# aai-institute/USFlows

Measured on AMD Instinct MI355X. Metric: log_prob samples/sec (whole node), 32-layer 784-dim flow, batch 65536, higher is better.
Workload: dtype f32 (GEMMs as bf16x3 split on the bf16 MFMA: 24 significant bits, fp32 accumulate); 1 GPU; BASELINE cfg2: USFlow in_dims=[784], 32 additive coupling blocks, ConditionalDenseNN[256, 256]+LeakyReLU(0.01), lu_transform=1, householder=0, affine_conjugation=False, Laplace(0,1) base; log_prob of 65536 rows per GPU (65536 over 1 GPU(s)) resident in HBM; conditioned synthetic parameters (seed 100, alpha 0.1); rows_per_gpu=65536, global_rows=65536, parallelism=dp1 (single GPU: no collective), fused_coupling=True, gemm_mode=bf16x3, merge_affine=auto -> False; probe (accepted, element-wise, L1) []

## Files before the change

### usflows_amd/csrc/usf_coupling_planes.hip

```cpp
#include <stdlib.h>

#include "usf_common.h"

namespace usf {

typedef __bf16 cp_bf16x8 __attribute__((ext_vector_type(8)));
typedef _Float16 cp_f16x8 __attribute__((ext_vector_type(8)));
#define USF_CP_F16_GUARD 65000.0f

template <int NPL> struct CPlanes;
template <> struct CPlanes<3> {
  typedef cp_bf16x8 vec;
  static __device__ __forceinline__ f32x4 mfma(vec a, vec b, f32x4 c) { return __builtin_amdgcn_mfma_f32_16x16x32_bf16(a, b, c, 0, 0, 0); }
  static __device__ __forceinline__ void split(const f32x4 x0, const f32x4 x1, vec (&o)[3]) {
#pragma unroll
    for (int j = 0; j < 8; ++j) {
      const float x = (j < 4) ? x0[j & 3] : x1[j & 3];
      const __bf16 h = (__bf16)x;
      const float r = x - (float)h;
      const __bf16 m = (__bf16)r;
      o[0][j] = h; o[1][j] = m; o[2][j] = (__bf16)(r - (float)m);
    }
  }
  static __device__ __forceinline__ void split1(const float x, const int j, vec (&o)[3]) {
    const __bf16 h = (__bf16)x;
    const float r = x - (float)h;
    const __bf16 m = (__bf16)r;
    o[0][j] = h; o[1][j] = m; o[2][j] = (__bf16)(r - (float)m);
  }
  static __device__ __forceinline__ void mm(f32x4& acc, const vec (&w)[3], const vec (&a)[3]) {
    acc = mfma(w[2], a[0], acc); acc = mfma(w[1], a[1], acc); acc = mfma(w[0], a[2], acc);
    acc = mfma(w[1], a[0], acc); acc = mfma(w[0], a[1], acc); acc = mfma(w[0], a[0], acc);
  }
};
template <> struct CPlanes<2> {
  typedef cp_f16x8 vec;
  static __device__ __forceinline__ f32x4 mfma(vec a, vec b, f32x4 c) { return __builtin_amdgcn_mfma_f32_16x16x32_f16(a, b, c, 0, 0, 0); }
  static __device__ __forceinline__ void split(const f32x4 x0, const f32x4 x1, vec (&o)[2]) {
#pragma unroll
    for (int j = 0; j < 8; ++j) {
      const float x = (j < 4) ? x0[j & 3] : x1[j & 3];
      const _Float16 h = (_Float16)x;
      o[0][j] = h; o[1][j] = (_Float16)(x - (float)h);
    }
  }
  static __device__ __forceinline__ void split1(const float x, const int j, vec (&o)[2]) {
    const _Float16 h = (_Float16)x;
    o[0][j] = h; o[1][j] = (_Float16)(x - (float)h);
  }
  static __device__ __forceinline__ void mm(f32x4& acc, const vec (&w)[2], const vec (&a)[2]) {
    acc = mfma(w[1], a[0], acc); acc = mfma(w[0], a[1], acc); acc = mfma(w[0], a[0], acc);
  }
};

struct CplPArgs {
  char* z; int z_nkb, npanels, M;
  int kb_p0, nk_p, kb_t0, nk_t;
  const char* Win; int64_t ld_in, pl_in; const float* b_in;
  const char* Whid[2]; int64_t ld_hid, pl_hid; const float* b_hid[2];
  const char* Wout; int64_t ld_out, pl_out; const float* b_out;
  float sign, slope; int act;
  int32_t* range_flag;
  unsigned long long* dbg;
  char* hout[2]; const char* gate[2];
  const float* ctx; int ctx_stride; const float* w_ctx; const float* b_ctx;
};

#ifdef USF_STAMP
#define CSTAMP(v) unsigned long long v = __builtin_amdgcn_s_memtime(); __builtin_amdgcn_sched_barrier(0)
#else
#define CSTAMP(v)
#endif

template <int NPL, int NH, int MODE = 0, bool CTX = false>
__global__ __launch_bounds__(512, 2) void coupling_planes_kernel(const CplPArgs p) {
  typedef CPlanes<NPL> PT;
  typedef typename PT::vec vec8;
  constexpr int T = 16;
  constexpr int HP = 16 * T;
  constexpr int KS = T / 2;
  constexpr int NT = 512;
  constexpr int SLOTS = NPL * 4 * HP;
  constexpr int NST = SLOTS / NT;
  constexpr int NPP = NST / NPL;
  constexpr int NC = HP / 8;
  constexpr int NPR = (NPL == 3) ? 6 : 3;
#ifndef USF_CP_AHEAD
#define USF_CP_AHEAD 3
#endif
  constexpr int AHEAD = USF_CP_AHEAD;
  __shared__ __attribute__((aligned(16))) float lds[2][SLOTS * 4];

  const int tid = threadIdx.x;
  const int lane = tid & 63;
  const int wave = tid >> 6;
  const int lj = lane & 15, lg = lane >> 4;
  const int panel = blockIdx.x * 8 + wave;
  const int panc = min(panel, p.npanels - 1);
  const bool live = panel < p.npanels;
  const bool live_z = CTX ? (live && 16 * panel + lj < p.M) : live;
  const f32x4 zero4 = {0.f, 0.f, 0.f, 0.f};
  constexpr unsigned CHB = NPL * 1024u;
  const size_t zbase = ((size_t)panc * p.z_nkb) * CHB + (size_t)lane * 16;

  int kdst[NPP];
  unsigned krow[NPP];
#pragma unroll
  for (int i = 0; i < NPP; ++i) {
    const int idx = tid + NT * i;
    const int r = idx >> 2, c = idx & 3;
    kdst[i] = 4 * (c * HP + (r ^ (2 * c)));
    krow[i] = (unsigned)r;
  }
  auto issue_k = [&](const char* W, int64_t ld, int64_t pl, int k0, f32x4 (&st)[NST]) {
#pragma unroll
    for (int q = 0; q < NPL; ++q)
#pragma unroll
      for (int i = 0; i < NPP; ++i)
        st[q * NPP + i] = *reinterpret_cast<const f32x4*>(W + 2 * (q * pl + (int64_t)krow[i] * ld + k0 + 8 * ((tid + NT * i) & 3)));
  };
  auto store_k = [&](int buf, const f32x4 (&st)[NST]) {
#pragma unroll
    for (int q = 0; q < NPL; ++q)
#pragma unroll
      for (int i = 0; i < NPP; ++i) *reinterpret_cast<f32x4*>(&lds[buf][q * 16 * HP + kdst[i]]) = st[q * NPP + i];
  };
  auto n_rc = [&](int i, int& r, int& c) { const int idx = tid + NT * i; r = idx / NC; c = idx % NC; };
  auto issue_n = [&](const char* W, int64_t ld, int64_t pl, int n0, f32x4 (&st)[NST]) {
#pragma unroll
    for (int q = 0; q < NPL; ++q)
#pragma unroll
      for (int i = 0; i < NPP; ++i) {
        int r, c; n_rc(i, r, c);
        st[q * NPP + i] = *reinterpret_cast<const f32x4*>(W + 2 * (q * pl + (int64_t)(n0 + r) * ld + 8 * c));
      }
  };
  auto store_n = [&](int buf, const f32x4 (&st)[NST]) {
#pragma unroll
    for (int q = 0; q < NPL; ++q)
#pragma unroll
      for (int i = 0; i < NPP; ++i) {
        int r, c; n_rc(i, r, c);
        *reinterpret_cast<f32x4*>(&lds[buf][4 * ((q * NC + c) * 32 + (r ^ (2 * (c & 7))))]) = st[q * NPP + i];
      }
  };

  f32x4 X1[T], X2[T];
#pragma unroll
  for (int t = 0; t < T; ++t) X1[t] = *reinterpret_cast<const f32x4*>(p.b_in + t * 16 + 4 * lg);
  if (CTX) {
// ... 221 lines not shown
#endif
  if (NPL == 2 && p.range_flag && bad && live && (16 * panel + lj) < p.M) atomicOr(p.range_flag, 1);
#undef CP_PIN_SLAB
}



#ifdef USF_STAMP
unsigned long long* g_cdbg = nullptr;
#endif

int coupling_planes_ctx(const usf_coupling_planes_desc* d, const float* ctx, int64_t ctx_stride, const float* w_ctx,
                        const float* b_ctx, hipStream_t stream) {
  if (!d) { set_error("usf_coupling_planes: null descriptor"); return -1; }
  if (ctx) {
    if (d->act == USF_ACT_GATE) { set_error("usf_coupling_planes_ctx: USF_ACT_GATE takes no context (the context enters no data gradient)"); return -2; }
    if (ctx_stride != 0 && ctx_stride != 1) { set_error("usf_coupling_planes_ctx: ctx_stride must be 0 or 1 (got %lld)", (long long)ctx_stride); return -2; }
    if (!w_ctx || !b_ctx || !aligned16(w_ctx) || !aligned16(b_ctx)) {
      set_error("usf_coupling_planes_ctx: w_ctx / b_ctx must be [256] fp32 vectors, 16-byte aligned");
      return -2;
    }
  }
  if (d->M < 0 || d->M > 0x7fffffff || d->z_nkb <= 0 || d->n_hidden < 1 || d->n_hidden > 3 || d->nk_p <= 0 || d->nk_t <= 0 ||
      d->kb_p0 < 0 || d->kb_t0 < 0 || d->kb_p0 + d->nk_p > d->z_nkb || d->kb_t0 + d->nk_t > d->z_nkb) {
    set_error("usf_coupling_planes: bad sizes / block ranges");
    return -2;
  }
  if (d->M == 0) return 0;
  if (d->format != USF_PLANES_BF16X3 && d->format != USF_PLANES_F16X2) { set_error("usf_coupling_planes: unknown format %d", d->format); return -2; }
  if (!d->z || !d->W_in || !d->W_out || !d->b_in || !d->b_out) { set_error("usf_coupling_planes: null pointer"); return -1; }
  for (int i = 0; i + 1 < d->n_hidden; ++i)
    if (!d->W_hid[i] || !d->b_hid[i]) { set_error("usf_coupling_planes: hidden layer %d missing", i); return -1; }
  if (d->hidden_padded != 256) { set_error("usf_coupling_planes: weights must be padded to a hidden width of 256 (got %d)", d->hidden_padded); return -2; }
  if (d->ldw_in < 32 * d->nk_p || (d->n_hidden > 1 && d->ldw_hid < 256) || d->ldw_out < 256 || (d->ldw_in & 7) || (d->ldw_hid & 7) ||
      (d->ldw_out & 7) || !aligned16(d->z) || !aligned16(d->W_in) || !aligned16(d->W_out) || !aligned16(d->b_in) || !aligned16(d->b_out)) {
    set_error("usf_coupling_planes: weight-image contract violated (ldw_in >= 32 nk_p, ldw_hid / ldw_out >= 256, multiples of 8, 16-byte aligned)");
    return -2;
  }
  const int64_t npl = d->format == USF_PLANES_F16X2 ? 2 : 3;
  const int64_t npanels = (d->M + 15) / 16;
  if (2 * npl * d->w_in_plane >= (1LL << 40)) { set_error("usf_coupling_planes: operand too large"); return -3; }
  CplPArgs a;
  a.z = reinterpret_cast<char*>(d->z); a.z_nkb = (int)d->z_nkb; a.npanels = (int)npanels; a.M = (int)d->M;
  a.kb_p0 = (int)d->kb_p0; a.nk_p = (int)d->nk_p; a.kb_t0 = (int)d->kb_t0; a.nk_t = (int)d->nk_t;
  a.Win = reinterpret_cast<const char*>(d->W_in); a.ld_in = d->ldw_in; a.pl_in = d->w_in_plane; a.b_in = d->b_in;
  for (int i = 0; i < 2; ++i) {
    const bool used = i + 1 < d->n_hidden;
    a.Whid[i] = reinterpret_cast<const char*>(used ? d->W_hid[i] : d->W_in);
    a.b_hid[i] = used ? d->b_hid[i] : d->b_in;
  }
  a.ld_hid = d->ldw_hid; a.pl_hid = d->w_hid_plane;
  a.Wout = reinterpret_cast<const char*>(d->W_out); a.ld_out = d->ldw_out; a.pl_out = d->w_out_plane; a.b_out = d->b_out;
  a.sign = d->sign; a.slope = d->slope; a.act = d->act; a.range_flag = d->range_flag;
  a.ctx = ctx; a.ctx_stride = (int)ctx_stride; a.w_ctx = w_ctx; a.b_ctx = b_ctx;
  a.dbg = nullptr;
#ifdef USF_STAMP
  a.dbg = g_cdbg;
#endif
  const dim3 grid((unsigned)((npanels + 7) / 8));
  const bool want_h = d->hidden_out[0] != nullptr || d->hidden_out[1] != nullptr;
  const bool gated = d->act == USF_ACT_GATE;
  if (d->act != USF_ACT_NONE && d->act != USF_ACT_LEAKY_RELU && !gated) { set_error("usf_coupling_planes: bad act %d", d->act); return -2; }
  for (int i = 0; i < 2; ++i) { a.hout[i] = nullptr; a.gate[i] = nullptr; }
  if (want_h || gated) {
    if (npl != 3 || d->n_hidden > 2) { set_error("usf_coupling_planes: hidden_out / USF_ACT_GATE need the bf16x3 format and n_hidden <= 2"); return -2; }
    if (gated && !want_h) { set_error("usf_coupling_planes: USF_ACT_GATE needs hidden_out (the gradients at the hidden pre-activations)"); return -2; }
    for (int i = 0; i < d->n_hidden; ++i) {
      if (!d->hidden_out[i] || !aligned16(d->hidden_out[i]) || (gated && (!d->gate[i] || !aligned16(d->gate[i])))) {
        set_error("usf_coupling_planes: hidden_out[l] (and gate[l] with USF_ACT_GATE) must be set for every hidden layer, 16-byte aligned");
        return -2;
      }
      a.hout[i] = reinterpret_cast<char*>(d->hidden_out[i]);
      a.gate[i] = reinterpret_cast<const char*>(gated ? d->gate[i] : nullptr);
    }
    const dim3 block(512);
#define USF_CPT(NH_, MODE_) hipLaunchKernelGGL((coupling_planes_kernel<3, NH_, MODE_>), grid, block, 0, stream, a)
#define USF_CPTC(NH_) hipLaunchKernelGGL((coupling_planes_kernel<3, NH_, 1, true>), grid, block, 0, stream, a)
    if (gated) { if (d->n_hidden == 1) USF_CPT(1, 2); else USF_CPT(2, 2); }
    else if (ctx) { if (d->n_hidden == 1) USF_CPTC(1); else USF_CPTC(2); }
    else { if (d->n_hidden == 1) USF_CPT(1, 1); else USF_CPT(2, 1); }
#undef USF_CPTC
#undef USF_CPT
    return check_launch("usf_coupling_planes");
  }
  const dim3 block(512);
#define USF_CPL(NPL_, NH_) hipLaunchKernelGGL((coupling_planes_kernel<NPL_, NH_>), grid, block, 0, stream, a)
#define USF_CPLC(NPL_, NH_) hipLaunchKernelGGL((coupling_planes_kernel<NPL_, NH_, 0, true>), grid, block, 0, stream, a)
  if (ctx) {
    if (npl == 2) {
      switch (d->n_hidden) { case 1: USF_CPLC(2, 1); break; case 2: USF_CPLC(2, 2); break; default: USF_CPLC(2, 3); break; }
    } else {
      switch (d->n_hidden) { case 1: USF_CPLC(3, 1); break; case 2: USF_CPLC(3, 2); break; default: USF_CPLC(3, 3); break; }
    }
  } else if (npl == 2) {
    switch (d->n_hidden) { case 1: USF_CPL(2, 1); break; case 2: USF_CPL(2, 2); break; default: USF_CPL(2, 3); break; }
  } else {
    switch (d->n_hidden) { case 1: USF_CPL(3, 1); break; case 2: USF_CPL(3, 2); break; default: USF_CPL(3, 3); break; }
  }
#undef USF_CPLC
#undef USF_CPL
  return check_launch("usf_coupling_planes");
}

int coupling_planes(const usf_coupling_planes_desc* d, hipStream_t stream) { return coupling_planes_ctx(d, nullptr, 0, nullptr, nullptr, stream); }

}
// ... 1 lines not shown
```

### usflows_amd/csrc/usf_planes.hip

```cpp
#include <stdlib.h>

#include "usf_common.h"

namespace usf {

typedef __bf16 bf16x8 __attribute__((ext_vector_type(8)));
typedef _Float16 f16x8 __attribute__((ext_vector_type(8)));
#define USF_F16_GUARD 65000.0f
#define USF_PL_LOAD_A(ptr) (*(ptr))
#define USF_PL_STORE_C(v, ptr) (*(ptr) = (v))

template <int NPL> struct Planes;
template <> struct Planes<3> {
  typedef bf16x8 vec;
  static __device__ __forceinline__ f32x4 mfma(vec a, vec b, f32x4 c) { return __builtin_amdgcn_mfma_f32_16x16x32_bf16(a, b, c, 0, 0, 0); }
  static __device__ __forceinline__ void split(const float (&x)[8], vec (&o)[3]) {
#pragma unroll
    for (int j = 0; j < 8; ++j) {
      const __bf16 h = (__bf16)x[j];
      const float r = x[j] - (float)h;
      const __bf16 m = (__bf16)r;
      const float r2 = r - (float)m;
      o[0][j] = h; o[1][j] = m; o[2][j] = (__bf16)r2;
    }
  }
};
template <> struct Planes<2> {
  typedef f16x8 vec;
  static __device__ __forceinline__ f32x4 mfma(vec a, vec b, f32x4 c) { return __builtin_amdgcn_mfma_f32_16x16x32_f16(a, b, c, 0, 0, 0); }
  static __device__ __forceinline__ void split(const float (&x)[8], vec (&o)[2]) {
#pragma unroll
    for (int j = 0; j < 8; ++j) {
      const _Float16 h = (_Float16)x[j];
      const float r = x[j] - (float)h;
      o[0][j] = h; o[1][j] = (_Float16)r;
    }
  }
};

__host__ __device__ __forceinline__ int plane_feature_of_slot(int s) { return 16 * ((s & 7) >> 2) + 4 * (s >> 3) + (s & 3); }

template <int NPL>
__global__ __launch_bounds__(256) void pack_planes_kernel(const float* __restrict__ src, int64_t ld, int M, int npanels,
                                                          int nkb, const int32_t* __restrict__ idx,
                                                          const float* __restrict__ pre_div,
                                                          const float* __restrict__ pre_sub, char* __restrict__ dst,
                                                          int32_t* __restrict__ range_flag) {
  typedef Planes<NPL> PT;
  const int lane = threadIdx.x & 63;
  const int lj = lane & 15, lg = lane >> 4;
  const int64_t chunk = (int64_t)blockIdx.x * 4 + (threadIdx.x >> 6);
  if (chunk >= (int64_t)npanels * nkb) return;
  const int p = (int)(chunk / nkb), kb = (int)(chunk % nkb);
  const int row = 16 * p + lj;
  float x[8];
#pragma unroll
  for (int u = 0; u < 8; ++u) {
    const int l = 32 * kb + 16 * (u >> 2) + 4 * lg + (u & 3);
    const int c = idx[l];
    float v = 0.f;
    if (c >= 0 && row < M) {
      v = src[(int64_t)row * ld + c];
      if (pre_div) v = v / pre_div[l];
      if (pre_sub) v = v - pre_sub[l];
    }
    x[u] = v;
  }
  if (NPL == 2 && range_flag) {
    bool bad = false;
#pragma unroll
    for (int u = 0; u < 8; ++u) bad = bad || !(fabsf(x[u]) < USF_F16_GUARD);
    if (bad) atomicOr(range_flag, 1);
  }
  typename PT::vec o[NPL];
  PT::split(x, o);
  char* out = dst + (chunk * NPL) * 1024 + lane * 16;
#pragma unroll
  for (int q = 0; q < NPL; ++q) *reinterpret_cast<typename PT::vec*>(out + q * 1024) = o[q];
}

template <int NPL, bool GRAD>
__global__ __launch_bounds__(256) void pack_planes_rows_kernel(const float* __restrict__ src, int64_t ld, int M, int nkb, int src_cols,
                                                               const int32_t* __restrict__ idx, const float* __restrict__ pre_div,
                                                               const float* __restrict__ pre_sub, char* __restrict__ dst,
                                                               int32_t* __restrict__ range_flag, const float* __restrict__ row_weight,
                                                               const float* __restrict__ loc, const float* __restrict__ scale, int grad_base,
                                                               int vec) {
  typedef Planes<NPL> PT;
  extern __shared__ float tile[];
  const int S = src_cols + 1;
  const int L = 32 * nkb;
  int* const t_idx = reinterpret_cast<int*>(tile + 16 * S);
  float* const t_div = tile + 16 * S + L;
  float* const t_sub = t_div + L;
  const int tid = threadIdx.x, lane = tid & 63, wave = tid >> 6;
  const int p = blockIdx.x;
  for (int e = tid; e < L; e += 256) {
    t_idx[e] = idx[e];
    t_div[e] = pre_div ? pre_div[e] : 1.0f;
    t_sub[e] = pre_sub ? pre_sub[e] : 0.0f;
  }
  auto xform = [&](float v, int c, float w) {
    if (!GRAD) return v;
    const float t = v - loc[c];
    const float sg = (float)((t > 0.f) - (t < 0.f));
    const float g = (grad_base == 1 + USF_BASE_LAPLACE) ? -sg / scale[c] : -t / (scale[c] * scale[c]);
    return g * w;
  };
  if (vec) {
    const int c4n = src_cols >> 2;
    for (int e = tid; e < 16 * c4n; e += 256) {
      const int r = e / c4n, c = 4 * (e - r * c4n);
      const int row = 16 * p + r;
      f32x4 v = {0.f, 0.f, 0.f, 0.f};
      float w = 0.f;
      if (row < M) {
        v = *reinterpret_cast<const f32x4*>(src + (int64_t)row * ld + c);
        if (GRAD) w = row_weight[row];
      }
#pragma unroll
      for (int q = 0; q < 4; ++q) tile[r * S + c + q] = (row < M) ? xform(v[q], c + q, w) : 0.f;
    }
    for (int e = tid; e < 16 * (src_cols & 3); e += 256) {
      const int r = e / (src_cols & 3), c = (src_cols & ~3) + e % (src_cols & 3);
      const int row = 16 * p + r;
      tile[r * S + c] = (row < M) ? xform(src[(int64_t)row * ld + c], c, GRAD ? row_weight[row] : 0.f) : 0.f;
    }
  } else {
    for (int e = tid; e < 16 * src_cols; e += 256) {
      const int r = e / src_cols, c = e - r * src_cols;
      const int row = 16 * p + r;
      tile[r * S + c] = (row < M) ? xform(src[(int64_t)row * ld + c], c, GRAD ? row_weight[row] : 0.f) : 0.f;
    }
  }
  __syncthreads();
  const int lj = lane & 15, lg = lane >> 4;
  const bool row_live = 16 * p + lj < M;
  const bool has_div = pre_div != nullptr, has_sub = pre_sub != nullptr;
  bool bad = false;
  for (int kb = wave; kb < nkb; kb += 4) {
    float x[8];
#pragma unroll
    for (int u = 0; u < 8; ++u) {
      const int l = 32 * kb + 16 * (u >> 2) + 4 * lg + (u & 3);
      const int c = t_idx[l];
      float v = 0.f;
      if (c >= 0 && row_live) {
        v = tile[lj * S + c];
        if (has_div) v = v / t_div[l];
        if (has_sub) v = v - t_sub[l];
      }
      x[u] = v;
    }
    if (NPL == 2) {
#pragma unroll
      for (int u = 0; u < 8; ++u) bad = bad || !(fabsf(x[u]) < USF_F16_GUARD);
    }
    typename PT::vec o[NPL];
    PT::split(x, o);
    char* out = dst + ((int64_t)((int64_t)p * nkb + kb) * NPL) * 1024 + lane * 16;
#pragma unroll
    for (int q = 0; q < NPL; ++q) *reinterpret_cast<typename PT::vec*>(out + q * 1024) = o[q];
  }
  if (NPL == 2 && range_flag && bad) atomicOr(range_flag, 1);
}

int pack_planes(const usf_pack_planes_desc* d, hipStream_t stream) {
  if (!d) { set_error("usf_pack_planes_f32: null descriptor"); return -1; }
  if (d->M < 0 || d->nkb <= 0 || d->M > 0x7fffffff || d->nkb > 0x7fffff || d->ld < 1) { set_error("usf_pack_planes_f32: bad sizes"); return -2; }
  if (d->M == 0) return 0;
  if (!d->src || !d->idx || !d->planes) { set_error("usf_pack_planes_f32: null pointer"); return -1; }
  if (!aligned16(d->planes)) { set_error("usf_pack_planes_f32: planes must be 16-byte aligned"); return -2; }
  if (d->format != USF_PLANES_BF16X3 && d->format != USF_PLANES_F16X2) { set_error("usf_pack_planes_f32: unknown format %d", d->format); return -2; }
  const int64_t npanels = (d->M + 15) / 16;
  const int64_t chunks = npanels * d->nkb;
  const int64_t blocks = (chunks + 3) / 4;
  if (blocks > 0x7fffffffLL) { set_error("usf_pack_planes_f32: grid too large"); return -3; }
  if (d->grad_base != 0) {
    if (d->src_cols <= 0 || !d->row_weight || !d->loc || !d->scale || d->format != USF_PLANES_BF16X3 ||
        (d->grad_base != 1 + USF_BASE_LAPLACE && d->grad_base != 1 + USF_BASE_NORMAL)) {
      set_error("usf_pack_planes_f32: grad_base needs src_cols, row_weight, loc, scale, the bf16x3 format and a Laplace / Normal base");
      return -2;
    }
  }
  const int rows_env = (int)tuning("pack_rows", 1);
  const size_t lds = ((size_t)16 * (size_t)(d->src_cols + 1) + (size_t)3 * 32 * (size_t)d->nkb) * sizeof(float);
  if (d->src_cols > 0 && d->src_cols <= d->ld && lds <= 65536 && (rows_env || d->grad_base != 0)) {
    const int vec = (aligned16(d->src) && (d->ld & 3) == 0) ? 1 : 0;
    char* out = reinterpret_cast<char*>(d->planes);
#define USF_PPR(NPL_, GRAD_) hipLaunchKernelGGL((pack_planes_rows_kernel<NPL_, GRAD_>), dim3((unsigned)npanels), dim3(256), lds, stream, d->src, \
                             d->ld, (int)d->M, (int)d->nkb, (int)d->src_cols, d->idx, d->pre_div, d->pre_sub, out, d->range_flag,      \
                             d->row_weight, d->loc, d->scale, (int)d->grad_base, vec)
    if (d->grad_base != 0) USF_PPR(3, true);
    else if (d->format == USF_PLANES_F16X2) USF_PPR(2, false);
    else USF_PPR(3, false);
#undef USF_PPR
    return check_launch("usf_pack_planes_f32");
  }
  if (d->grad_base != 0) { set_error("usf_pack_planes_f32: grad_base needs 16 (src_cols + 1) floats to fit 64 KB of LDS"); return -2; }
  if (d->format == USF_PLANES_F16X2)
    hipLaunchKernelGGL(pack_planes_kernel<2>, dim3((unsigned)blocks), dim3(256), 0, stream, d->src, d->ld, (int)d->M, (int)npanels,
                       (int)d->nkb, d->idx, d->pre_div, d->pre_sub, reinterpret_cast<char*>(d->planes), d->range_flag);
  else
    hipLaunchKernelGGL(pack_planes_kernel<3>, dim3((unsigned)blocks), dim3(256), 0, stream, d->src, d->ld, (int)d->M, (int)npanels,
                       (int)d->nkb, d->idx, d->pre_div, d->pre_sub, reinterpret_cast<char*>(d->planes), d->range_flag);
  return check_launch("usf_pack_planes_f32");
}

struct PlArgs {
  const char* A; const char* Wp; const float* bias; const float* post_mul;
  const char* R; char* Cp; float* Cf;
  int64_t ldc, plane_stride;
  int ldwp, wrows;
  int M, npanels;
  int a_nkb, a_kb0, nk;
  int c_nkb, c_kb0, c_kbn;
  int N, nbm, nbn, nvb;
  float res_sign, slope; int act;
  int32_t* range_flag;
  const float* b_tab; float* b_part; int b_stride; int b_base;
  unsigned long long* clk;
  unsigned long long* dbg;
  unsigned long long* span;
};

template <int NPL, int TN, bool F32OUT>
__global__ __launch_bounds__(512, 2) void gemm_planes_kernel(const PlArgs p) {
  typedef Planes<NPL> PT;
  typedef typename PT::vec vec8;
  constexpr int NT = 512;
  constexpr int BN = TN * 32;
  constexpr int FT = 2 * TN;
  constexpr unsigned CHB = NPL * 1024u;
  constexpr int CS = BN;
  constexpr int NSLOT = NPL * 4 * BN;
  constexpr int NWV = (NSLOT + NT - 1) / NT;
  constexpr int STG = NPL * 4 * CS * 4;
  constexpr int NB = 3;
  static_assert(NWV * NT - NSLOT <= NSLOT, "surplus threads wrap once");
  __shared__ __attribute__((aligned(16))) float wring[NB * STG];

  const int tid = threadIdx.x;
  const int lane = tid & 63;
  const int wave = tid >> 6;
  const int lj = lane & 15, lg = lane >> 4;
#ifdef USF_STAMP
  if (p.span && tid == 0) atomicMin(p.span, __builtin_amdgcn_s_memrealtime());
#endif
  unsigned long long clk_c0 = 0, clk_r0 = 0;
#ifndef USF_NO_CLOCK
  if (p.clk) { clk_c0 = __builtin_amdgcn_s_memtime(); clk_r0 = __builtin_amdgcn_s_memrealtime(); }
#endif

  for (int bid = blockIdx.x; bid < p.nvb; bid += gridDim.x) {
  const int xcd = bid & 7;
  const int seq = bid >> 3;
  const int pg = (seq / p.nbn) * 8 + xcd;
  const int bn = seq % p.nbn;
  if (pg >= p.nbm) continue;
  if (bid != (int)blockIdx.x) __syncthreads();
  const int n0 = bn * BN;
  int pw[2];
  pw[0] = pg * 16 + wave * 2;
  pw[1] = pw[0] + 1;

  unsigned aoff[2];
#pragma unroll
  for (int b = 0; b < 2; ++b)
    aoff[b] = ((unsigned)min(pw[b], p.npanels - 1) * (unsigned)p.a_nkb + (unsigned)p.a_kb0) * CHB + (unsigned)lane * 16u;
  auto issue_a = [&](int kb, vec8 (&dst)[2][NPL]) {
#pragma unroll
    for (int b = 0; b < 2; ++b)
#pragma unroll
      for (int q = 0; q < NPL; ++q)
        dst[b][q] = USF_PL_LOAD_A(reinterpret_cast<const vec8*>(p.A + (aoff[b] + (unsigned)kb * CHB + (unsigned)q * 1024u)));
  };

  unsigned wsrc[NWV];
  int wdst[NWV];
#pragma unroll
  for (int i = 0; i < NWV; ++i) {
    const int idx = tid + NT * i;
    const int idc = (idx < NSLOT) ? idx : idx - NSLOT;
    const int pl = idc / (4 * BN), rem = idc % (4 * BN);
    const int r = rem >> 2, ch = rem & 3;
    wsrc[i] = (unsigned)(2 * (pl * p.plane_stride + (int64_t)min(n0 + r, p.wrows - 1) * p.ldwp + 8 * ch));
    wdst[i] = 4 * ((pl * 4 + ch) * CS + (r ^ (2 * ch)));
  }
  auto issue_w = [&](int k0, f32x4 (&dst)[NWV]) {
#pragma unroll
    for (int i = 0; i < NWV; ++i) dst[i] = *reinterpret_cast<const f32x4*>(p.Wp + (wsrc[i] + 2u * (unsigned)k0));
  };
  auto store_w = [&](float* wb, const f32x4 (&src)[NWV]) {
#pragma unroll
    for (int i = 0; i < NWV; ++i) *reinterpret_cast<f32x4*>(wb + wdst[i]) = src[i];
  };

  f32x4 acc[FT][2];
  const f32x4 zero4 = {0.f, 0.f, 0.f, 0.f};
#pragma unroll
  for (int ft = 0; ft < FT; ++ft) {
    f32x4 bv = zero4;
    if (p.bias) bv = *reinterpret_cast<const f32x4*>(p.bias + min(n0 + ft * 16 + 4 * lg, p.wrows - 4));
    acc[ft][0] = bv;
    acc[ft][1] = bv;
  }

#ifdef USF_STAMP
#define PSTAMP(v) unsigned long long v = __builtin_amdgcn_s_memtime(); __builtin_amdgcn_sched_barrier(0)
#else
#define PSTAMP(v)
#endif
  PSTAMP(t0);
#ifdef USF_STAMP
  const unsigned long long rt0 = __builtin_amdgcn_s_memrealtime();
#endif
  vec8 pa[2][NPL], pb[2][NPL];
  vec8 fr[2][NPL], f2[2][NPL];
  f32x4 wst[NWV];
  const int nslab = p.nk;
  auto ks = [&](int s_) { return s_; };
  issue_w(ks(0) * 32, wst);
  store_w(wring, wst);
  issue_a(ks(0), pa);
  issue_w(ks(min(1, nslab - 1)) * 32, wst);
  __syncthreads();
  const float* const wl0 = wring + 4 * (lg * CS + (lj ^ (2 * lg)));
  auto read_pair = [&](const float* wl, int pr, vec8 (&f)[2][NPL]) {
#pragma unroll
    for (int q = 0; q < NPL; ++q) {
      f[0][q] = *reinterpret_cast<const vec8*>(wl + 4 * (q * 4 * CS + (2 * pr) * 16));
      f[1][q] = *reinterpret_cast<const vec8*>(wl + 4 * (q * 4 * CS + (2 * pr + 1) * 16));
    }
  };
  read_pair(wl0, 0, fr);

  constexpr int NPR = (NPL == 3) ? 6 : 3;
  constexpr int NP = TN;
  constexpr int MID = (NP - 1) / 2;
  constexpr int NLD = 2 * NPL;
  constexpr int LPP = (NLD + MID) / (MID + 1);
#define USF_MM(FT_, W, P)                                        \
  acc[FT_][0] = PT::mfma(W, cur[0][P], acc[FT_][0]);             \
  acc[FT_][1] = PT::mfma(W, cur[1][P], acc[FT_][1])
  auto mm_pair = [&](int pr, const vec8 (&f)[2][NPL], const vec8 (&cur)[2][NPL]) {
    const int ft = 2 * pr;
    if (NPL == 3) {
      USF_MM(ft, f[0][2], 0); USF_MM(ft + 1, f[1][2], 0); USF_MM(ft, f[0][1], 1); USF_MM(ft + 1, f[1][1], 1);
      USF_MM(ft, f[0][0], NPL - 1); USF_MM(ft + 1, f[1][0], NPL - 1); USF_MM(ft, f[0][1], 0); USF_MM(ft + 1, f[1][1], 0);
      USF_MM(ft, f[0][0], 1); USF_MM(ft + 1, f[1][0], 1); USF_MM(ft, f[0][0], 0); USF_MM(ft + 1, f[1][0], 0);
    } else {
      USF_MM(ft, f[0][1], 0); USF_MM(ft + 1, f[1][1], 0); USF_MM(ft, f[0][0], 1); USF_MM(ft + 1, f[1][0], 1);
      USF_MM(ft, f[0][0], 0); USF_MM(ft + 1, f[1][0], 0);
    }
  };
#if defined(USF_STAMP) && USF_STAMP >= 2
  unsigned long long ph[4] = {0, 0, 0, 0};
#define LSTAMP(v) PSTAMP(v)
#define LACC(i, a, b) ph[i] += (b) - (a)
#else
#define LSTAMP(v)
#define LACC(i, a, b)
#endif
  auto slab = [&](int s, int ring_s, const vec8 (&cur)[2][NPL], vec8 (&nxt)[2][NPL], vec8 (&fA)[2][NPL], vec8 (&fB)[2][NPL]) {
    LSTAMP(l0);
    const int ring_n = (ring_s == 2) ? 0 : ring_s + 1;
    const float* wl = wl0 + ring_s * STG;
    const float* wln = wl0 + ring_n * STG;
    float* wb = wring + ring_n * STG;
    issue_a(ks(min(s + 1, nslab - 1)), nxt);
#pragma unroll
    for (int pr = 0; pr <= MID; ++pr) {
      if (pr & 1) { if (pr + 1 < NP) read_pair(wl, pr + 1, fA); mm_pair(pr, fB, cur); }
      else        { if (pr + 1 < NP) read_pair(wl, pr + 1, fB); mm_pair(pr, fA, cur); }
      if (pr == MID) store_w(wb, wst);
      __builtin_amdgcn_sched_group_barrier(0x100, 2 * NPL, 0);
      if (pr < MID) {
        __builtin_amdgcn_sched_group_barrier(0x008, 2 * NPR, 0);
        if (pr * LPP < NLD) __builtin_amdgcn_sched_group_barrier(0x020, LPP, 0);
        __builtin_amdgcn_sched_group_barrier(0x008, 2 * NPR, 0);
      } else {
        constexpr int MPS = (4 * NPR) / (NWV + 1);
#pragma unroll
        for (int i = 0; i < NWV; ++i) {
          __builtin_amdgcn_sched_group_barrier(0x008, MPS, 0);
          __builtin_amdgcn_sched_group_barrier(0x200, 1, 0);
        }
        __builtin_amdgcn_sched_group_barrier(0x008, 4 * NPR - NWV * MPS, 0);
      }
    }
    __builtin_amdgcn_sched_barrier(0);
    LSTAMP(l1);
    LSTAMP(l2);
    __syncthreads();
    __builtin_amdgcn_sched_barrier(0);
    LSTAMP(l3);
    issue_w(ks(min(s + 2, nslab - 1)) * 32, wst);
#pragma unroll
    for (int pr = MID + 1; pr < NP; ++pr) {
      if (pr & 1) { if (pr + 1 < NP) read_pair(wl, pr + 1, fA); else read_pair(wln, 0, fA); mm_pair(pr, fB, cur); }
      else        { if (pr + 1 < NP) read_pair(wl, pr + 1, fB); else read_pair(wln, 0, fB); mm_pair(pr, fA, cur); }
      __builtin_amdgcn_sched_group_barrier(0x100, 2 * NPL, 0);
      if (pr == MID + 1) {
        __builtin_amdgcn_sched_group_barrier(0x008, 2 * NPR, 0);
        __builtin_amdgcn_sched_group_barrier(0x020, NWV, 0);
        __builtin_amdgcn_sched_group_barrier(0x008, 2 * NPR, 0);
      } else {
        __builtin_amdgcn_sched_group_barrier(0x008, 4 * NPR, 0);
      }
    }
    __builtin_amdgcn_sched_barrier(0);
    LSTAMP(l4);
    LACC(0, l0, l1); LACC(1, l1, l2); LACC(2, l2, l3); LACC(3, l3, l4);
  };
  PSTAMP(t1);
  int s = 0, ring = 0;
  for (; s + 2 <= nslab; s += 2) {
    slab(s, ring, pa, pb, fr, f2);
    ring = (ring == 2) ? 0 : ring + 1;
    if (NP & 1) slab(s + 1, ring, pb, pa, f2, fr); else slab(s + 1, ring, pb, pa, fr, f2);
    ring = (ring == 2) ? 0 : ring + 1;
  }
  if (s < nslab) slab(s, ring, pa, pb, fr, f2);
#undef USF_MM
  PSTAMP(t2);

  bool bad = false;
  if (p.act == USF_ACT_LEAKY_RELU) {
#pragma unroll
    for (int ft = 0; ft < FT; ++ft)
#pragma unroll
      for (int b = 0; b < 2; ++b)
#pragma unroll
        for (int j = 0; j < 4; ++j) acc[ft][b][j] = act_apply(acc[ft][b][j], USF_ACT_LEAKY_RELU, p.slope);
  }
  if (F32OUT) {
    const bool vec_ok = ((p.ldc & 3) == 0) && ((reinterpret_cast<uintptr_t>(p.Cf) & 15u) == 0);
#pragma unroll
    for (int b = 0; b < 2; ++b) {
      const int row = 16 * pw[b] + lj;
      float bsum = 0.f;
#pragma unroll
      for (int ft = 0; ft < FT; ++ft) {
        const int col = n0 + 16 * ft + 4 * lg;
        f32x4 v = acc[ft][b];
        if (p.post_mul) v = v * *reinterpret_cast<const f32x4*>(p.post_mul + min(col, p.wrows - 4));
        if (p.b_part) {
          const float* t = p.b_tab + min(col, p.b_stride - 4);
          const f32x4 bl = *reinterpret_cast<const f32x4*>(t);
          const f32x4 bi = *reinterpret_cast<const f32x4*>(t + p.b_stride);
          const f32x4 bc = *reinterpret_cast<const f32x4*>(t + 2 * p.b_stride);
#pragma unroll
          for (int j = 0; j < 4; ++j) {
            const float d = (v[j] - bl[j]) * bi[j];
            const float term = (p.b_base == USF_BASE_LAPLACE) ? bc[j] - fabsf(d) : bc[j] - 0.5f * d * d;
            bsum += (col + j < p.N) ? term : 0.f;
          }
        }
        if (NPL == 2 && row < p.M && col < p.N) {
#pragma unroll
          for (int j = 0; j < 4; ++j) bad = bad || (col + j < p.N && !(fabsf(v[j]) < 3.0e38f));
        }
        if (p.Cf != nullptr && row < p.M && col < p.N) {
          float* dst = p.Cf + (int64_t)row * p.ldc + col;
          if (vec_ok && col + 3 < p.N) {
            *reinterpret_cast<f32x4*>(dst) = v;
          } else {
#pragma unroll
            for (int j = 0; j < 4; ++j)
              if (col + j < p.N) dst[j] = v[j];
          }
        }
      }
      if (p.b_part) {
        bsum += __shfl_xor(bsum, 16);
        bsum += __shfl_xor(bsum, 32);
        if (lg == 0 && row < p.M) p.b_part[(int64_t)row * 8 + bn] = bsum;
// ... 1 lines not shown
    }
  } else {
#pragma unroll
    for (int t = 0; t < TN; ++t) {
      const int kbo = bn * TN + t;
#pragma unroll
      for (int b = 0; b < 2; ++b) {
        if (kbo < p.c_kbn && pw[b] < p.npanels) {
          const size_t off = (((size_t)pw[b] * p.c_nkb + (p.c_kb0 + kbo)) * NPL) * 1024 + (size_t)lane * 16;
          float x[8];
#pragma unroll
          for (int u = 0; u < 8; ++u) x[u] = acc[2 * t + (u >> 2)][b][u & 3];
          if (p.R) {
            vec8 r[NPL];
#pragma unroll
            for (int q = 0; q < NPL; ++q) r[q] = *reinterpret_cast<const vec8*>(p.R + off + q * 1024);
#pragma unroll
            for (int u = 0; u < 8; ++u) {
              float rv = (float)r[0][u] + (float)r[1][u];
              if (NPL == 3) rv = rv + (float)r[NPL - 1][u];
              x[u] = rv + p.res_sign * x[u];
            }
          }
          if (NPL == 2) {
#pragma unroll
            for (int u = 0; u < 8; ++u) bad = bad || (16 * pw[b] + lj < p.M && !(fabsf(x[u]) < USF_F16_GUARD));
          }
          vec8 o[NPL];
          PT::split(x, o);
#ifdef USF_NOSTORE
          if (o[0][0] == (decltype(o[0][0] + o[0][0]))1234.5f && o[1][1] == (decltype(o[0][0] + o[0][0]))77.f)
#endif
          {
#pragma unroll
            for (int q = 0; q < NPL; ++q) USF_PL_STORE_C(o[q], reinterpret_cast<vec8*>(p.Cp + off + q * 1024));
          }
        }
      }
    }
  }
  if (NPL == 2 && p.range_flag && bad) atomicOr(p.range_flag, 1);
#ifdef USF_STAMP
  PSTAMP(t3);
  if (p.dbg && lane == 0) {
    unsigned long long* o = p.dbg + (size_t)((bid % 2048) * 8 + wave) * 8;
    o[0] = t1 - t0; o[1] = t2 - t1; o[2] = t3 - t2; o[3] = t3 - t0; o[4] = 1; o[5] = __builtin_amdgcn_s_memrealtime() - rt0;
    o[6] = rt0; o[7] = __builtin_amdgcn_s_memrealtime();
#if USF_STAMP >= 2
    unsigned long long* o2 = p.dbg + 16384 * 8 + (size_t)((bid % 2048) * 8 + wave) * 8;
    for (int i = 0; i < 4; ++i) o2[i] = ph[i];
#endif
  }
#endif
  }
#ifdef USF_STAMP
  if (p.span && tid == 0) atomicMax(p.span + 1, __builtin_amdgcn_s_memrealtime());
#endif
#ifndef USF_NO_CLOCK
  if (p.clk && tid == 0) {
    atomicAdd(p.clk, __builtin_amdgcn_s_memtime() - clk_c0);
    atomicAdd(p.clk + 1, __builtin_amdgcn_s_memrealtime() - clk_r0);
  }
#endif
}

#ifdef USF_STAMP
unsigned long long* g_pdbg = nullptr;
unsigned long long* g_pspan = nullptr;
#endif

template <int NPL, int TN>
static int launch_planes(PlArgs a, bool f32out, hipStream_t stream) {
  constexpr int BN = TN * 32;
  a.nbm = (a.npanels + 15) / 16;
  a.nbn = f32out ? (a.N + BN - 1) / BN : (a.c_kbn + TN - 1) / TN;
  int64_t grid = (((int64_t)a.nbm + 7) / 8) * 8 * a.nbn;
  if (grid > 0x7fffffffLL) { set_error("usf_gemm_planes: grid too large"); return -3; }
  a.nvb = (int)grid;
  const int persist = (int)tuning("planes_persist", 1);
  int cus = device_cu_count();
  cus = (cus / 8) * 8 > 0 ? (cus / 8) * 8 : 8;
  if (persist && grid > cus) grid = cus;
  if (f32out) hipLaunchKernelGGL((gemm_planes_kernel<NPL, TN, true>), dim3((unsigned)grid), dim3(512), 0, stream, a);
  else hipLaunchKernelGGL((gemm_planes_kernel<NPL, TN, false>), dim3((unsigned)grid), dim3(512), 0, stream, a);
  return check_launch("usf_gemm_planes");
}

int gemm_planes_tn(int64_t nblk) {
  const int64_t pad5 = (nblk + 4) / 5 * 5 - nblk, pad4 = (nblk + 3) / 4 * 4 - nblk;
  return pad4 < pad5 ? 4 : 5;
}

int gemm_planes_variant(const usf_gemm_planes_desc* d) {
  if (!d || d->M <= 0) return 0;
  const bool f32out = d->C_f32 != nullptr || d->base_part != nullptr;
  const int64_t nblk = f32out ? (d->N + 31) / 32 : d->c_kbn;
  if (nblk <= 0) return 0;
  return 5000 + 10 * gemm_planes_tn(nblk) + (f32out ? 1 : 0);
}

int gemm_planes(const usf_gemm_planes_desc* d, hipStream_t stream) {
  if (!d) { set_error("usf_gemm_planes_bf16x3: null descriptor"); return -1; }
  if (d->M < 0 || d->M > 0x7fffffff || d->nk <= 0 || d->a_nkb <= 0 || d->a_kb0 < 0 || d->a_kb0 + d->nk > d->a_nkb ||
      d->w_rows < 4 || d->w_rows > 0x7fffffff) {
    set_error("usf_gemm_planes_bf16x3: bad sizes (M=%lld nk=%lld a_nkb=%lld a_kb0=%lld w_rows=%lld)", (long long)d->M,
              (long long)d->nk, (long long)d->a_nkb, (long long)d->a_kb0, (long long)d->w_rows);
    return -2;
  }
  if (d->M == 0) return 0;
  const bool f32out = d->C_f32 != nullptr || d->base_part != nullptr;
  if (!d->A || !d->W_planes || (!f32out && !d->C_planes)) { set_error("usf_gemm_planes_bf16x3: null A / W / C"); return -1; }
  if (f32out && d->C_planes) { set_error("usf_gemm_planes_bf16x3: give C_planes or C_f32, not both"); return -2; }
  if (!aligned16(d->A) || !aligned16(d->W_planes) || (d->C_planes && !aligned16(d->C_planes)) ||
      (d->residual && !aligned16(d->residual)) || (d->bias && !aligned16(d->bias)) || (d->post_mul && !aligned16(d->post_mul))) {
    set_error("usf_gemm_planes_bf16x3: pointers must be 16-byte aligned");
    return -2;
  }
  if ((d->ldw & 7) || d->ldw < 32 * d->nk || (d->w_rows & 3)) { set_error("usf_gemm_planes_bf16x3: ldw must be a multiple of 8 and >= 32 nk; w_rows a multiple of 4"); return -2; }
  if (d->act != USF_ACT_NONE && d->act != USF_ACT_LEAKY_RELU) { set_error("usf_gemm_planes_bf16x3: bad act"); return -2; }
  const int64_t npanels = (d->M + 15) / 16;
  if (d->format != USF_PLANES_BF16X3 && d->format != USF_PLANES_F16X2) { set_error("usf_gemm_planes_bf16x3: unknown format %d", d->format); return -2; }
  const int64_t npl = d->format == USF_PLANES_F16X2 ? 2 : 3;
  if (npanels * d->a_nkb * npl * 1024 >= (1LL << 32) || 2 * npl * d->w_plane_stride >= (1LL << 32)) {
    set_error("usf_gemm_planes_bf16x3: operand larger than the kernel's 32-bit offsets");
    return -3;
  }
  PlArgs a;
  a.A = reinterpret_cast<const char*>(d->A); a.Wp = reinterpret_cast<const char*>(d->W_planes);
  a.bias = d->bias; a.post_mul = d->post_mul; a.R = reinterpret_cast<const char*>(d->residual);
  a.Cp = reinterpret_cast<char*>(d->C_planes); a.Cf = d->C_f32; a.ldc = d->ldc; a.plane_stride = d->w_plane_stride;
  a.ldwp = (int)d->ldw; a.wrows = (int)d->w_rows; a.M = (int)d->M; a.npanels = (int)npanels;
  a.a_nkb = (int)d->a_nkb; a.a_kb0 = (int)d->a_kb0; a.nk = (int)d->nk;
  a.c_nkb = (int)d->c_nkb; a.c_kb0 = (int)d->c_kb0; a.c_kbn = (int)d->c_kbn; a.N = (int)d->N;
  a.res_sign = d->res_sign; a.slope = d->slope; a.act = d->act; a.nbm = a.nbn = a.nvb = 0;
  a.range_flag = d->range_flag;
  a.b_tab = d->base_tab; a.b_part = d->base_part; a.b_stride = (int)d->base_tab_stride; a.b_base = d->base;
  a.dbg = nullptr; a.span = nullptr;
  a.clk = clock_buffer();
#ifdef USF_STAMP
  a.dbg = g_pdbg; a.span = g_pspan;
  if (g_pspan) g_pspan += 2;
#endif
  int64_t nblk;
  if (f32out) {
    if (d->N <= 0 || d->N > d->w_rows || d->ldc < d->N) { set_error("usf_gemm_planes_bf16x3: bad N / ldc for fp32 output"); return -2; }
    if (d->residual) { set_error("usf_gemm_planes_bf16x3: residual needs planes output"); return -2; }
    nblk = (d->N + 31) / 32;
    if (d->base_part) {
      if (!d->base_tab || !aligned16(d->base_tab) || (d->base_tab_stride & 3) || d->base_tab_stride < ((d->N + 3) & ~(int64_t)3) ||
          d->base_tab_stride > 0x7fffffff || (d->base != USF_BASE_LAPLACE && d->base != USF_BASE_NORMAL)) {
        set_error("usf_gemm_planes_bf16x3: base density in the epilogue needs the tables of usf_base_tables_f32 (16-byte aligned, "
                  "stride a multiple of 4 and >= N) and base = USF_BASE_LAPLACE / USF_BASE_NORMAL");
        return -2;
      }
    }
  } else {
    if (d->base_part) { set_error("usf_gemm_planes_bf16x3: base_part needs the fp32-output form"); return -2; }
    if (d->c_kbn <= 0 || d->c_kb0 < 0 || d->c_kb0 + d->c_kbn > d->c_nkb || d->c_kbn * 32 > d->w_rows) {
      set_error("usf_gemm_planes_bf16x3: bad output block range (c_kb0=%lld c_kbn=%lld c_nkb=%lld w_rows=%lld)",
                (long long)d->c_kb0, (long long)d->c_kbn, (long long)d->c_nkb, (long long)d->w_rows);
      return -2;
    }
    if (npanels * d->c_nkb * npl * 1024 >= (1LL << 40)) { set_error("usf_gemm_planes_bf16x3: output too large"); return -3; }
    nblk = d->c_kbn;
  }
  const int force = (int)tuning("planes_tn", 0);
  const int tn = (force == 4 || force == 5) ? force : gemm_planes_tn(nblk);
  if (d->base_part && (d->N + 32 * tn - 1) / (32 * tn) > 8) {
    set_error("usf_gemm_planes_bf16x3: base_part holds 8 column blocks per row (N <= 1024)");
    return -2;
  }
  if (npl == 2) return tn == 4 ? launch_planes<2, 4>(a, f32out, stream) : launch_planes<2, 5>(a, f32out, stream);
  return tn == 4 ? launch_planes<3, 4>(a, f32out, stream) : launch_planes<3, 5>(a, f32out, stream);
}

}
```

Before: 3.517 million samples/s.

## Skip zero-padded weight tiles, widen pack kernel, reverse coupling block order

Three independent changes. The planes GEMM scans the last N-block's final 16 weight rows at runtime, and when they are all zero (padding) it runs a specialised tile that skips the half-pair of MFMAs and LDS reads for them. The row-packing kernel gains a 512-thread variant, selected by default. The coupling kernel can walk panels in reverse block order, also on by default, presumably to favour cache or tail behaviour. The dead-row scan adds global reads per block and doubles the tile code through two instantiations.

```diff
diff --git a/usflows_amd/csrc/usf_coupling_planes.hip b/usflows_amd/csrc/usf_coupling_planes.hip
--- a/usflows_amd/csrc/usf_coupling_planes.hip
+++ b/usflows_amd/csrc/usf_coupling_planes.hip
@@ -61,6 +61,7 @@
   const char* Wout; int64_t ld_out, pl_out; const float* b_out;
   float sign, slope; int act;
   int32_t* range_flag;
+  int descend;
   unsigned long long* dbg;
   char* hout[2]; const char* gate[2];
   const float* ctx; int ctx_stride; const float* w_ctx; const float* b_ctx;
@@ -95,7 +96,7 @@
   const int lane = tid & 63;
   const int wave = tid >> 6;
   const int lj = lane & 15, lg = lane >> 4;
-  const int panel = blockIdx.x * 8 + wave;
+  const int panel = (p.descend ? (int)(gridDim.x - 1 - blockIdx.x) : (int)blockIdx.x) * 8 + wave;
   const int panc = min(panel, p.npanels - 1);
   const bool live = panel < p.npanels;
   const bool live_z = CTX ? (live && 16 * panel + lj < p.M) : live;
@@ -423,6 +424,7 @@
   a.ld_hid = d->ldw_hid; a.pl_hid = d->w_hid_plane;
   a.Wout = reinterpret_cast<const char*>(d->W_out); a.ld_out = d->ldw_out; a.pl_out = d->w_out_plane; a.b_out = d->b_out;
   a.sign = d->sign; a.slope = d->slope; a.act = d->act; a.range_flag = d->range_flag;
+  a.descend = (int)tuning("coupling_descend", 1);
   a.ctx = ctx; a.ctx_stride = (int)ctx_stride; a.w_ctx = w_ctx; a.b_ctx = b_ctx;
   a.dbg = nullptr;
 #ifdef USF_STAMP
diff --git a/usflows_amd/csrc/usf_planes.hip b/usflows_amd/csrc/usf_planes.hip
--- a/usflows_amd/csrc/usf_planes.hip
+++ b/usflows_amd/csrc/usf_planes.hip
@@ -1,4 +1,6 @@
 #include <stdlib.h>
+
+#include <type_traits>
 
 #include "usf_common.h"
 
@@ -6,6 +8,7 @@
 
 typedef __bf16 bf16x8 __attribute__((ext_vector_type(8)));
 typedef _Float16 f16x8 __attribute__((ext_vector_type(8)));
+typedef unsigned u32x4 __attribute__((ext_vector_type(4)));
 #define USF_F16_GUARD 65000.0f
 #define USF_PL_LOAD_A(ptr) (*(ptr))
 #define USF_PL_STORE_C(v, ptr) (*(ptr) = (v))
@@ -79,8 +82,8 @@
   for (int q = 0; q < NPL; ++q) *reinterpret_cast<typename PT::vec*>(out + q * 1024) = o[q];
 }
 
-template <int NPL, bool GRAD>
-__global__ __launch_bounds__(256) void pack_planes_rows_kernel(const float* __restrict__ src, int64_t ld, int M, int nkb, int src_cols,
+template <int NPL, bool GRAD, int NT>
+__global__ __launch_bounds__(NT) void pack_planes_rows_kernel(const float* __restrict__ src, int64_t ld, int M, int nkb, int src_cols,
                                                                const int32_t* __restrict__ idx, const float* __restrict__ pre_div,
                                                                const float* __restrict__ pre_sub, char* __restrict__ dst,
                                                                int32_t* __restrict__ range_flag, const float* __restrict__ row_weight,
@@ -95,7 +98,7 @@
   float* const t_sub = t_div + L;
   const int tid = threadIdx.x, lane = tid & 63, wave = tid >> 6;
   const int p = blockIdx.x;
-  for (int e = tid; e < L; e += 256) {
+  for (int e = tid; e < L; e += NT) {
     t_idx[e] = idx[e];
     t_div[e] = pre_div ? pre_div[e] : 1.0f;
     t_sub[e] = pre_sub ? pre_sub[e] : 0.0f;
@@ -109,7 +112,7 @@
   };
   if (vec) {
     const int c4n = src_cols >> 2;
-    for (int e = tid; e < 16 * c4n; e += 256) {
+    for (int e = tid; e < 16 * c4n; e += NT) {
       const int r = e / c4n, c = 4 * (e - r * c4n);
       const int row = 16 * p + r;
       f32x4 v = {0.f, 0.f, 0.f, 0.f};
@@ -121,13 +124,13 @@
 #pragma unroll
       for (int q = 0; q < 4; ++q) tile[r * S + c + q] = (row < M) ? xform(v[q], c + q, w) : 0.f;
     }
-    for (int e = tid; e < 16 * (src_cols & 3); e += 256) {
+    for (int e = tid; e < 16 * (src_cols & 3); e += NT) {
       const int r = e / (src_cols & 3), c = (src_cols & ~3) + e % (src_cols & 3);
       const int row = 16 * p + r;
       tile[r * S + c] = (row < M) ? xform(src[(int64_t)row * ld + c], c, GRAD ? row_weight[row] : 0.f) : 0.f;
     }
   } else {
-    for (int e = tid; e < 16 * src_cols; e += 256) {
+    for (int e = tid; e < 16 * src_cols; e += NT) {
       const int r = e / src_cols, c = e - r * src_cols;
       const int row = 16 * p + r;
       tile[r * S + c] = (row < M) ? xform(src[(int64_t)row * ld + c], c, GRAD ? row_weight[row] : 0.f) : 0.f;
@@ -138,7 +141,7 @@
   const bool row_live = 16 * p + lj < M;
   const bool has_div = pre_div != nullptr, has_sub = pre_sub != nullptr;
   bool bad = false;
-  for (int kb = wave; kb < nkb; kb += 4) {
+  for (int kb = wave; kb < nkb; kb += NT / 64) {
     float x[8];
 #pragma unroll
     for (int u = 0; u < 8; ++u) {
@@ -188,12 +191,15 @@
   if (d->src_cols > 0 && d->src_cols <= d->ld && lds <= 65536 && (rows_env || d->grad_base != 0)) {
     const int vec = (aligned16(d->src) && (d->ld & 3) == 0) ? 1 : 0;
     char* out = reinterpret_cast<char*>(d->planes);
-#define USF_PPR(NPL_, GRAD_) hipLaunchKernelGGL((pack_planes_rows_kernel<NPL_, GRAD_>), dim3((unsigned)npanels), dim3(256), lds, stream, d->src, \
-                             d->ld, (int)d->M, (int)d->nkb, (int)d->src_cols, d->idx, d->pre_div, d->pre_sub, out, d->range_flag,      \
+    const int wide = (int)tuning("pack_wide", 1);
+#define USF_PPR(NPL_, GRAD_, NT_) hipLaunchKernelGGL((pack_planes_rows_kernel<NPL_, GRAD_, NT_>), dim3((unsigned)npanels), dim3(NT_), lds, stream, \
+                             d->src, d->ld, (int)d->M, (int)d->nkb, (int)d->src_cols, d->idx, d->pre_div, d->pre_sub, out, d->range_flag,  \
                              d->row_weight, d->loc, d->scale, (int)d->grad_base, vec)
-    if (d->grad_base != 0) USF_PPR(3, true);
-    else if (d->format == USF_PLANES_F16X2) USF_PPR(2, false);
-    else USF_PPR(3, false);
+#define USF_PPW(NPL_, GRAD_) do { if (wide) USF_PPR(NPL_, GRAD_, 512); else USF_PPR(NPL_, GRAD_, 256); } while (0)
+    if (d->grad_base != 0) USF_PPW(3, true);
+    else if (d->format == USF_PLANES_F16X2) USF_PPW(2, false);
+    else USF_PPW(3, false);
+#undef USF_PPW
 #undef USF_PPR
     return check_launch("usf_pack_planes_f32");
   }
@@ -218,6 +224,7 @@
   int N, nbm, nbn, nvb;
   float res_sign, slope; int act;
   int32_t* range_flag;
+  int skip_dead;
   const float* b_tab; float* b_part; int b_stride; int b_base;
   unsigned long long* clk;
   unsigned long long* dbg;
@@ -240,19 +247,21 @@
   static_assert(NWV * NT - NSLOT <= NSLOT, "surplus threads wrap once");
   __shared__ __attribute__((aligned(16))) float wring[NB * STG];
 
-  const int tid = threadIdx.x;
+  const int tid0 = threadIdx.x;
+#ifdef USF_STAMP
+  if (p.span && tid0 == 0) atomicMin(p.span, __builtin_amdgcn_s_memrealtime());
+#endif
+  unsigned long long clk_c0 = 0, clk_r0 = 0;
+#ifndef USF_NO_CLOCK
+  if (p.clk) { clk_c0 = __builtin_amdgcn_s_memtime(); clk_r0 = __builtin_amdgcn_s_memrealtime(); }
+#endif
+
+  for (int bid = blockIdx.x; bid < p.nvb; bid += gridDim.x) {
+  int tid = tid0;
+  asm volatile("" : "+v"(tid));
   const int lane = tid & 63;
   const int wave = tid >> 6;
   const int lj = lane & 15, lg = lane >> 4;
-#ifdef USF_STAMP
-  if (p.span && tid == 0) atomicMin(p.span, __builtin_amdgcn_s_memrealtime());
-#endif
-  unsigned long long clk_c0 = 0, clk_r0 = 0;
-#ifndef USF_NO_CLOCK
-  if (p.clk) { clk_c0 = __builtin_amdgcn_s_memtime(); clk_r0 = __builtin_amdgcn_s_memrealtime(); }
-#endif
-
-  for (int bid = blockIdx.x; bid < p.nvb; bid += gridDim.x) {
   const int xcd = bid & 7;
   const int seq = bid >> 3;
   const int pg = (seq / p.nbn) * 8 + xcd;
@@ -264,6 +273,27 @@
   pw[0] = pg * 16 + wave * 2;
   pw[1] = pw[0] + 1;
 
+  bool dead = false;
+  if (p.skip_dead && bn == p.nbn - 1 && n0 + BN <= p.wrows) {
+    const int spr = 4 * p.nk;
+    const int nscan = NPL * 16 * spr;
+    const char* const wz = p.Wp + 2 * ((int64_t)(n0 + BN - 16) * p.ldwp);
+    unsigned nz = 0;
+    for (int e0 = tid; e0 < nscan; e0 += 4 * NT) {
+      u32x4 v[4];
+#pragma unroll
+      for (int i = 0; i < 4; ++i) {
+        const int e = min(e0 + i * NT, nscan - 1);
+        const int pl = e / (16 * spr), rem = e - pl * (16 * spr);
+        const int r = rem / spr, c = rem - r * spr;
+        v[i] = *reinterpret_cast<const u32x4*>(wz + 2 * (pl * p.plane_stride + (int64_t)r * p.ldwp + 8 * c));
+      }
+#pragma unroll
+      for (int i = 0; i < 4; ++i) nz |= v[i][0] | v[i][1] | v[i][2] | v[i][3];
+    }
+    dead = __builtin_amdgcn_readfirstlane(__syncthreads_or(nz != 0)) == 0;
+  }
+  auto tile = [&](auto dead_c) {
   unsigned aoff[2];
 #pragma unroll
   for (int b = 0; b < 2; ++b)
@@ -333,6 +363,10 @@
       f[1][q] = *reinterpret_cast<const vec8*>(wl + 4 * (q * 4 * CS + (2 * pr + 1) * 16));
     }
   };
+  auto read_half = [&](const float* wl, int pr, vec8 (&f)[2][NPL]) {
+#pragma unroll
+    for (int q = 0; q < NPL; ++q) f[0][q] = *reinterpret_cast<const vec8*>(wl + 4 * (q * 4 * CS + (2 * pr) * 16));
+  };
   read_pair(wl0, 0, fr);
 
   constexpr int NPR = (NPL == 3) ? 6 : 3;
@@ -343,9 +377,17 @@
 #define USF_MM(FT_, W, P)                                        \
   acc[FT_][0] = PT::mfma(W, cur[0][P], acc[FT_][0]);             \
   acc[FT_][1] = PT::mfma(W, cur[1][P], acc[FT_][1])
-  auto mm_pair = [&](int pr, const vec8 (&f)[2][NPL], const vec8 (&cur)[2][NPL]) {
+  static_assert(NP - 1 > MID + 1, "the last pair runs behind the barrier and carries no global loads");
+  auto mm_pair = [&](auto dead_c, int pr, const vec8 (&f)[2][NPL], const vec8 (&cur)[2][NPL]) {
     const int ft = 2 * pr;
-    if (NPL == 3) {
+    if (decltype(dead_c)::value && pr == NP - 1) {
+      if constexpr (NPL == 3) {
+        USF_MM(ft, f[0][2], 0); USF_MM(ft, f[0][1], 1); USF_MM(ft, f[0][0], NPL - 1); USF_MM(ft, f[0][1], 0);
+        USF_MM(ft, f[0][0], 1); USF_MM(ft, f[0][0], 0);
+      } else {
+        USF_MM(ft, f[0][1], 0); USF_MM(ft, f[0][0], 1); USF_MM(ft, f[0][0], 0);
+      }
+    } else if constexpr (NPL == 3) {
       USF_MM(ft, f[0][2], 0); USF_MM(ft + 1, f[1][2], 0); USF_MM(ft, f[0][1], 1); USF_MM(ft + 1, f[1][1], 1);
       USF_MM(ft, f[0][0], NPL - 1); USF_MM(ft + 1, f[1][0], NPL - 1); USF_MM(ft, f[0][1], 0); USF_MM(ft + 1, f[1][1], 0);
       USF_MM(ft, f[0][0], 1); USF_MM(ft + 1, f[1][0], 1); USF_MM(ft, f[0][0], 0); USF_MM(ft + 1, f[1][0], 0);
@@ -362,17 +404,21 @@
 #define LSTAMP(v)
 #define LACC(i, a, b)
 #endif
-  auto slab = [&](int s, int ring_s, const vec8 (&cur)[2][NPL], vec8 (&nxt)[2][NPL], vec8 (&fA)[2][NPL], vec8 (&fB)[2][NPL]) {
+  auto slab = [&](auto dead_c, int s, int ring_s, const vec8 (&cur)[2][NPL], vec8 (&nxt)[2][NPL], vec8 (&fA)[2][NPL], vec8 (&fB)[2][NPL]) {
+    constexpr bool DEAD = decltype(dead_c)::value;
     LSTAMP(l0);
     const int ring_n = (ring_s == 2) ? 0 : ring_s + 1;
     const float* wl = wl0 + ring_s * STG;
     const float* wln = wl0 + ring_n * STG;
+    auto read_next = [&](int pr, vec8 (&f)[2][NPL]) {
+      if (DEAD && pr + 1 == NP - 1) read_half(wl, pr + 1, f); else read_pair(wl, pr + 1, f);
+    };
     float* wb = wring + ring_n * STG;
     issue_a(ks(min(s + 1, nslab - 1)), nxt);
 #pragma unroll
     for (int pr = 0; pr <= MID; ++pr) {
-      if (pr & 1) { if (pr + 1 < NP) read_pair(wl, pr + 1, fA); mm_pair(pr, fB, cur); }
-      else        { if (pr + 1 < NP) read_pair(wl, pr + 1, fB); mm_pair(pr, fA, cur); }
+      if (pr & 1) { if (pr + 1 < NP) read_next(pr, fA); mm_pair(dead_c, pr, fB, cur); }
+      else        { if (pr + 1 < NP) read_next(pr, fB); mm_pair(dead_c, pr, fA, cur); }
       if (pr == MID) store_w(wb, wst);
       __builtin_amdgcn_sched_group_barrier(0x100, 2 * NPL, 0);
       if (pr < MID) {
@@ -398,13 +444,16 @@
     issue_w(ks(min(s + 2, nslab - 1)) * 32, wst);
 #pragma unroll
     for (int pr = MID + 1; pr < NP; ++pr) {
-      if (pr & 1) { if (pr + 1 < NP) read_pair(wl, pr + 1, fA); else read_pair(wln, 0, fA); mm_pair(pr, fB, cur); }
-      else        { if (pr + 1 < NP) read_pair(wl, pr + 1, fB); else read_pair(wln, 0, fB); mm_pair(pr, fA, cur); }
-      __builtin_amdgcn_sched_group_barrier(0x100, 2 * NPL, 0);
+      if (pr & 1) { if (pr + 1 < NP) read_next(pr, fA); else read_pair(wln, 0, fA); mm_pair(dead_c, pr, fB, cur); }
+      else        { if (pr + 1 < NP) read_next(pr, fB); else read_pair(wln, 0, fB); mm_pair(dead_c, pr, fA, cur); }
+      if (DEAD && pr + 1 == NP - 1) __builtin_amdgcn_sched_group_barrier(0x100, NPL, 0);
+      else __builtin_amdgcn_sched_group_barrier(0x100, 2 * NPL, 0);
       if (pr == MID + 1) {
         __builtin_amdgcn_sched_group_barrier(0x008, 2 * NPR, 0);
         __builtin_amdgcn_sched_group_barrier(0x020, NWV, 0);
         __builtin_amdgcn_sched_group_barrier(0x008, 2 * NPR, 0);
+      } else if (DEAD && pr == NP - 1) {
+        __builtin_amdgcn_sched_group_barrier(0x008, 2 * NPR, 0);
       } else {
         __builtin_amdgcn_sched_group_barrier(0x008, 4 * NPR, 0);
       }
@@ -414,15 +463,14 @@
     LACC(0, l0, l1); LACC(1, l1, l2); LACC(2, l2, l3); LACC(3, l3, l4);
   };
   PSTAMP(t1);
-  int s = 0, ring = 0;
-  for (; s + 2 <= nslab; s += 2) {
-    slab(s, ring, pa, pb, fr, f2);
-    ring = (ring == 2) ? 0 : ring + 1;
-    if (NP & 1) slab(s + 1, ring, pb, pa, f2, fr); else slab(s + 1, ring, pb, pa, fr, f2);
-    ring = (ring == 2) ? 0 : ring + 1;
-  }
-  if (s < nslab) slab(s, ring, pa, pb, fr, f2);
-#undef USF_MM
+    int s = 0, ring = 0;
+    for (; s + 2 <= nslab; s += 2) {
+      slab(dead_c, s, ring, pa, pb, fr, f2);
+      ring = (ring == 2) ? 0 : ring + 1;
+      if (NP & 1) slab(dead_c, s + 1, ring, pb, pa, f2, fr); else slab(dead_c, s + 1, ring, pb, pa, fr, f2);
+      ring = (ring == 2) ? 0 : ring + 1;
+    }
+    if (s < nslab) slab(dead_c, s, ring, pa, pb, fr, f2);
   PSTAMP(t2);
 
   bool bad = false;
@@ -530,12 +578,15 @@
 #endif
   }
 #endif
+  };
+  if (dead) tile(std::true_type()); else tile(std::false_type());
+#undef USF_MM
   }
 #ifdef USF_STAMP
-  if (p.span && tid == 0) atomicMax(p.span + 1, __builtin_amdgcn_s_memrealtime());
+  if (p.span && tid0 == 0) atomicMax(p.span + 1, __builtin_amdgcn_s_memrealtime());
 #endif
 #ifndef USF_NO_CLOCK
-  if (p.clk && tid == 0) {
+  if (p.clk && tid0 == 0) {
     atomicAdd(p.clk, __builtin_amdgcn_s_memtime() - clk_c0);
     atomicAdd(p.clk + 1, __builtin_amdgcn_s_memrealtime() - clk_r0);
   }
@@ -612,6 +663,7 @@
   a.c_nkb = (int)d->c_nkb; a.c_kb0 = (int)d->c_kb0; a.c_kbn = (int)d->c_kbn; a.N = (int)d->N;
   a.res_sign = d->res_sign; a.slope = d->slope; a.act = d->act; a.nbm = a.nbn = a.nvb = 0;
   a.range_flag = d->range_flag;
+  a.skip_dead = (int)tuning("planes_skip_dead", 1);
   a.b_tab = d->base_tab; a.b_part = d->base_part; a.b_stride = (int)d->base_tab_stride; a.b_base = d->base;
   a.dbg = nullptr; a.span = nullptr;
   a.clk = clock_buffer();
```

After: 3.594 million samples/s, median of 6. +2.2%, better.
